# zkHubHQ/distributed-groth16

Hardware: NVIDIA H100
Metric: G1 MSM throughput (BN254 Pippenger, 2^20 pairs per GPU) (higher is better)
Workload: dtype u32x8 Montgomery (256-bit modular integers)

## Files before the change

### distributed_groth16_b200/csrc/ec.cuh

```cuda
#pragma once
#include "fp.cuh"

namespace b200zk {

template <class F>
struct affine_t {
    F x, y;
    B2_HD bool is_inf() const { return x.is_zero() && y.is_zero(); }
    B2_HD static affine_t infinity() { affine_t r; r.x = F::zero(); r.y = F::zero(); return r; }
};

template <class F>
struct xyzz_t {
    F x, y, zz, zzz;

    B2_HD static xyzz_t identity() {
        xyzz_t r; r.x = F::zero(); r.y = F::zero(); r.zz = F::zero(); r.zzz = F::zero(); return r;
    }
    B2_HD bool is_inf() const { return zz.is_zero(); }

    B2_HD static xyzz_t from_affine(const affine_t<F>& p) {
        if (p.is_inf()) return identity();
        xyzz_t r; r.x = p.x; r.y = p.y; r.zz = F::one(); r.zzz = F::one(); return r;
    }
// ... 138 lines not shown
        return r;
    }
    B2_HD_NI static affine_t<F> to_affine(const xyzz_t& a) {
        if (a.is_inf()) return affine_t<F>::infinity();
        return to_affine(a, F::inv(a.zzz));
    }

    B2_HD_NI static xyzz_t mul_scalar(const xyzz_t& p, const uint32_t k[8]) {
        xyzz_t acc = identity();
        for (int bit = 255; bit >= 0; --bit) {
            acc = dbl(acc);
            if ((k[bit >> 5] >> (bit & 31)) & 1) acc = add(acc, p);
        }
        return acc;
    }
};

template <class F> B2_HD affine_t<F> curve_generator();
template <> B2_HD affine_t<Fq> curve_generator<Fq>() {
    affine_t<Fq> g;
    for (int i = 0; i < 8; ++i) { g.x.l[i] = CurveConst::g1_gen_x(i); g.y.l[i] = CurveConst::g1_gen_y(i); }
    return g;
}
template <> B2_HD affine_t<Fq2> curve_generator<Fq2>() {
    affine_t<Fq2> g;
    for (int i = 0; i < 8; ++i) {
        g.x.c0.l[i] = CurveConst::g2_gen_x0(i); g.x.c1.l[i] = CurveConst::g2_gen_x1(i);
        g.y.c0.l[i] = CurveConst::g2_gen_y0(i); g.y.c1.l[i] = CurveConst::g2_gen_y1(i);
    }
    return g;
}

#ifdef __CUDACC__
template <class F, bool FULLWARP = false>
struct quad_ops {
    static constexpr int WORDS = sizeof(F) / 4;

    __device__ __forceinline__ static unsigned quad_mask() { return FULLWARP ? 0xFFFFFFFFu : (0xFu << (threadIdx.x & 28u)); }
    __device__ __forceinline__ static int quad_lane() { return threadIdx.x & 3; }

    struct xch_t { F p[2][4]; };
    __device__ __forceinline__ static F sel(int q, const F& a0, const F& a1, const F& a2, const F& a3) {
        F r;
        const uint32_t* p0 = reinterpret_cast<const uint32_t*>(&a0);
        const uint32_t* p1 = reinterpret_cast<const uint32_t*>(&a1);
        const uint32_t* p2 = reinterpret_cast<const uint32_t*>(&a2);
        const uint32_t* p3 = reinterpret_cast<const uint32_t*>(&a3);
        uint32_t* pr = reinterpret_cast<uint32_t*>(&r);
#pragma unroll
        for (int i = 0; i < WORDS; ++i) pr[i] = q == 0 ? p0[i] : q == 1 ? p1[i] : q == 2 ? p2[i] : p3[i];
        return r;
    }
    __device__ __forceinline__ static void mul4(xch_t* x, int buf, const F& a0, const F& b0, const F& a1, const F& b1,
                                                const F& a2, const F& b2, const F& a3, const F& b3, F& p0, F& p1, F& p2, F& p3) {
        const int q = quad_lane();
        F a = sel(q, a0, a1, a2, a3), b = sel(q, b0, b1, b2, b3);
        F p = F::mul(a, b);
        st16(&x->p[buf][q], p);
        __syncwarp(quad_mask());
        p0 = ld16(&x->p[buf][0]); p1 = ld16(&x->p[buf][1]); p2 = ld16(&x->p[buf][2]); p3 = ld16(&x->p[buf][3]);
    }

    __device__ static xyzz_t<F> dbl(xch_t* x, const xyzz_t<F>& p) {
        if (p.is_inf()) return p;
        F U = F::dbl(p.y);
        F V, X2, d0, d1;
        mul4(x, 0, U, U, p.x, p.x, U, U, U, U, V, X2, d0, d1);
        F M = F::add(F::dbl(X2), X2);
        F W, S, ZZ3, MM;
        mul4(x, 1, U, V, p.x, V, V, p.zz, M, M, W, S, ZZ3, MM);
        xyzz_t<F> r;
        r.x = F::sub(MM, F::dbl(S));
        F T1, T2, ZZZ3;
        mul4(x, 0, M, F::sub(S, r.x), W, p.y, W, p.zzz, W, W, T1, T2, ZZZ3, d0);
        r.y = F::sub(T1, T2);
        r.zz = ZZ3;
        r.zzz = ZZZ3;
        __syncwarp(quad_mask());
        return r;
    }

    __device__ static xyzz_t<F> add(xch_t* x, const xyzz_t<F>& a, const xyzz_t<F>& b) {
        if (a.is_inf()) return b;
        if (b.is_inf()) return a;
        F U1, U2, S1, S2;
        mul4(x, 0, a.x, b.zz, b.x, a.zz, a.y, b.zzz, b.y, a.zzz, U1, U2, S1, S2);
        F Pp = F::sub(U2, U1), R = F::sub(S2, S1);
        if (Pp.is_zero()) {
            __syncwarp(quad_mask());
            if (R.is_zero()) return dbl(x, a);
            return xyzz_t<F>::identity();
        }
        F PP, RR, ZZ12, ZZZ12;
        mul4(x, 1, Pp, Pp, R, R, a.zz, b.zz, a.zzz, b.zzz, PP, RR, ZZ12, ZZZ12);
        F PPP, Q, ZZ3, d0;
        mul4(x, 0, Pp, PP, U1, PP, ZZ12, PP, PP, PP, PPP, Q, ZZ3, d0);
        xyzz_t<F> r;
        r.x = F::sub(F::sub(RR, PPP), F::dbl(Q));
        F T1, T2, ZZZ3;
        mul4(x, 1, R, F::sub(Q, r.x), S1, PPP, ZZZ12, PPP, PPP, PPP, T1, T2, ZZZ3, d0);
        r.y = F::sub(T1, T2);
        r.zz = ZZ3;
        r.zzz = ZZZ3;
        __syncwarp(quad_mask());
        return r;
    }
};
#endif

struct G1Curve {
    typedef Fq F;
    static constexpr int LIMBS64 = 8;
};
struct G2Curve {
    typedef Fq2 F;
    static constexpr int LIMBS64 = 16;
};

}
```

### distributed_groth16_b200/csrc/msm.cu

```cuda
#include "common.cuh"
#include "glv.cuh"

namespace b200zk {

static const uint32_t KEY_NONE = 0xFFFFFFFFu;

__global__ void k_msm_digits(const Fr* scalars, uint32_t n, uint32_t c, uint32_t W, uint32_t* keys, uint32_t* ranks,
                             uint32_t* counts) {
    uint32_t i = blockIdx.x * blockDim.x + threadIdx.x;
    if (i >= n) return;
    Fr s = Fr::from_mont(ld16(scalars + i));
    uint32_t k[9];
#pragma unroll
    for (int j = 0; j < 8; ++j) k[j] = s.l[j];
    k[8] = 0;
    const uint32_t B = 1u << (c - 1);
    const uint32_t mask = (1u << c) - 1;
    uint32_t carry = 0;
    for (uint32_t w = 0; w < W; ++w) {
        uint32_t off = w * c, limb = off >> 5, sh = off & 31;
        uint64_t v = limb < 8 ? ((uint64_t)k[limb] | ((uint64_t)k[limb + 1] << 32)) : 0;
        uint32_t d = ((uint32_t)(v >> sh) & mask) + carry;
        uint32_t key = KEY_NONE, rank = 0;
        carry = 0;
        uint32_t neg = 0;
        if (d > B) { d = (1u << c) - d; neg = 1; carry = 1; }
        if (d != 0) {
            uint32_t g = d - 1;
            rank = atomicAdd(counts + g, 1u);
            key = g | (neg << 31);
        }
        const size_t slot = (size_t)w * n + i;
        keys[slot] = key;
        ranks[slot] = rank;
// ... 288 lines not shown
        run = Q::add(x, run, ld16(bw + k));
        acc = Q::add(x, acc, run);
    }
    if (lo) {
        xyzz_t<F> m = xyzz_t<F>::identity();
        for (int bit = 31 - __clz(lo); bit >= 0; --bit) {
            m = Q::dbl(x, m);
            if ((lo >> bit) & 1) m = Q::add(x, m, run);
        }
        acc = Q::add(x, acc, m);
    }
    if ((threadIdx.x & 3) == 0) st16(partials + t, acc);
}

template <class F, int THREADS>
__global__ void __launch_bounds__(THREADS) k_msm_window_sum(const xyzz_t<F>* partials, uint32_t nseg, xyzz_t<F>* wsum) {
    __shared__ xyzz_t<F> sh[THREADS];
    const xyzz_t<F>* p = partials + (size_t)blockIdx.x * nseg;
    xyzz_t<F> acc = xyzz_t<F>::identity();
    for (uint32_t i = threadIdx.x; i < nseg; i += THREADS) acc = add_sel<F>(acc, ld16(p + i));
    sh[threadIdx.x] = acc;
    __syncthreads();
    for (int s = THREADS / 2; s > 0; s >>= 1) {
        if ((int)threadIdx.x < s) {
            xyzz_t<F> a = sh[threadIdx.x], b = sh[threadIdx.x + s];
            sh[threadIdx.x] = add_sel<F>(a, b);
        }
        __syncthreads();
    }
    if (threadIdx.x == 0) st16(wsum + blockIdx.x, sh[0]);
}

template <class F>
__global__ void __launch_bounds__(32) k_msm_horner(const xyzz_t<F>* wsum, uint32_t nset, uint32_t c, uint32_t first, uint32_t last,
                                                   xyzz_t<F>* state, xyzz_t<F>* out) {
    typedef quad_ops<F, false> Q;
    __shared__ typename Q::xch_t xch;
    if (blockIdx.x != 0 || threadIdx.x >= 4) return;
    xyzz_t<F> total;
    uint32_t k = 0;
    if (first) { total = ld16(wsum); k = 1; }
    else total = ld16(state);
    for (; k < nset; ++k) {
        for (uint32_t j = 0; j < c; ++j) total = Q::dbl(&xch, total);
        total = Q::add(&xch, total, ld16(wsum + k));
    }
    if (threadIdx.x == 0) st16(last ? out : state, total);
}

template <class F>
__global__ void __launch_bounds__(32) k_msm_horner_glv(const xyzz_t<F>* wsum, uint32_t nwin, uint32_t c, uint32_t first, uint32_t last,
                                                       xyzz_t<F>* state, xyzz_t<F>* out) {
    typedef quad_ops<F, false> Q;
    __shared__ typename Q::xch_t xch[2];
    __shared__ xyzz_t<F> h1;
    if (blockIdx.x != 0 || threadIdx.x >= 8) return;
    const uint32_t half = threadIdx.x >> 2;
    xyzz_t<F> total;
    uint32_t k = 0;
    if (first) { total = ld16(wsum + half); k = 1; }
    else total = ld16(state + half);
    for (; k < nwin; ++k) {
        for (uint32_t j = 0; j < c; ++j) total = Q::dbl(&xch[half], total);
        total = Q::add(&xch[half], total, ld16(wsum + 2 * k + half));
    }
    if (!last) {
        if ((threadIdx.x & 3) == 0) st16(state + half, total);
        return;
    }
    if (threadIdx.x == 4) h1 = total;
    __syncwarp(0xFFu);
    if (half == 0) {
        xyzz_t<F> p = h1;
        if (!p.is_inf()) glv_phi_x(p.x);
        total = Q::add(&xch[0], total, p);
        if (threadIdx.x == 0) st16(out, total);
    }
}

template <class F>
__global__ void k_sum_to_affine(const xyzz_t<F>* pts, uint32_t count, affine_t<F>* out, uint64_t* flag) {
    if (threadIdx.x != 0 || blockIdx.x != 0) return;
    xyzz_t<F> acc = xyzz_t<F>::identity();
    for (uint32_t i = 0; i < count; ++i) acc = xyzz_t<F>::add(acc, ld16(pts + i));
    affine_t<F> a = xyzz_t<F>::to_affine(acc);
    st16(out, a);
    *flag = acc.is_inf() ? 1 : 0;
}

template <class F>
__global__ void k_set_identity(xyzz_t<F>* out) {
    if (threadIdx.x == 0 && blockIdx.x == 0) st16(out, xyzz_t<F>::identity());
}

static unsigned choose_window(size_t n) {
    unsigned lg = ceil_log2(n < 2 ? 2 : n);
    int c = (int)lg - 4;
    if (c < 5) c = 5;
    if (c > 20) c = 20;
    const char* env = getenv("B200ZK_MSM_WINDOW");
    if (env) { int v = atoi(env); if (v >= 2 && v <= 24) c = v; }
    return (unsigned)c;
}

// ... 39 lines not shown
template <class F>
static int msm_dev_impl(b200zk_ctx* ctx, const MsmStreams& ms, DevBuf& ws_buf, const MsmPart* parts, unsigned nparts,
                        void* d_out, const char* acc_name, unsigned tab_c = 0) {
    const int ch = ms.channel;
    size_t nev = 0;
    auto next_event = [&]() { return msm_event(ctx, ch, nev++); };
    size_t n = 0, n_max = 0;
    for (unsigned p = 0; p < nparts; ++p) { n += parts[p].n; n_max = parts[p].n > n_max ? parts[p].n : n_max; }
    xyzz_t<F>* out = reinterpret_cast<xyzz_t<F>*>(d_out);
    if (n == 0) {
        {
            LaunchScope ls(ctx, ms.acc, "msm_small");
            k_set_identity<F><<<1, 32, 0, ms.acc>>>(out);
        }
        return check_launch(ctx, "k_set_identity");
    }
    if (n >= (1ull << 31)) return set_error(ctx, B200ZK_ERR_ARG, "MSM length must be < 2^31");
    const bool fold = tab_c != 0;
    if (fold && nparts != 1) return set_error(ctx, B200ZK_ERR_ARG, "fixed-base tables take one input part");
    const unsigned c = fold ? tab_c : choose_window(n);
    const unsigned Wh = (128 + c - 1) / c;
    const unsigned W = fold ? msm_table_windows(c) : 2 * Wh;
    const unsigned WB = fold ? 1 : W;
    if ((uint64_t)W * n >= (fold ? (1ull << 31) : (1ull << 32)))
        return set_error(ctx, B200ZK_ERR_ARG, "MSM too large for 32-bit bucket offsets / entry indices (W * n)");
    const uint32_t B = 1u << (c - 1);
    const uint32_t nb = WB * B;
    uint32_t seg_len = B < 16 ? B : 16;
    const bool quad_reduce = (uint64_t)WB * (B / seg_len) <= 8192;
    if (quad_reduce) seg_len = B < 8 ? B : 8;
    else if (ctx->msm_seg_hint && ctx->msm_seg_hint <= B) seg_len = ctx->msm_seg_hint;
    const uint32_t nseg = B / seg_len;
    const uint32_t wsplit = fold ? (nseg >= 16 * 256 ? 16 : (nseg >= 1024 ? 4 : 1)) : 1;

    const unsigned unit_sets = fold ? 1 : 2;
    const unsigned units = fold ? 1 : Wh;
    unsigned ngroups = 1;
    if (!fold && nparts == 1 && n >= (1u << 22)) ngroups = units < 4 ? units : 4;
    auto group_first_unit = [&](unsigned g) { return (unsigned)(((uint64_t)units * g) / ngroups); };
    const uint32_t rmw = nparts > 1 ? 1u : 0u;

    const bool split_streams = ngroups > 1 || nparts > 1;
    const cudaStream_t st = split_streams ? ms.seq : ms.acc, ast = ms.acc;
    if (split_streams) {
        cudaEvent_t e = next_event();
        if (!e) return set_error(ctx, B200ZK_ERR_CUDA, "cudaEventCreate failed");
        B2_CUDA_OK(ctx, cudaEventRecord(e, ast));
        B2_CUDA_OK(ctx, cudaStreamWaitEvent(st, e, 0));
    }
    auto finish = [&]() -> int {
        if (split_streams) {
            cudaEvent_t e = next_event();
            if (!e) return set_error(ctx, B200ZK_ERR_CUDA, "cudaEventCreate failed");
            B2_CUDA_OK(ctx, cudaEventRecord(e, st));
            B2_CUDA_OK(ctx, cudaStreamWaitEvent(ast, e, 0));
        }
        return B200ZK_OK;
    };

    auto al = [](size_t x) { return (x + 255) & ~(size_t)255; };
    const size_t total_max = (size_t)W * n_max;
    uint32_t task_len = TASK_LEN;
    while (task_len < MAX_TASK_LEN && (uint64_t)task_len * nb < 3 * (uint64_t)total_max &&
           total_max / (2 * task_len) + nb >= (1u << 19))
        task_len *= 2;
    if (n_max <= (1u << 16))
        while (task_len > 16 && total_max / task_len < (1u << 17)) task_len /= 2;
    const size_t max_tasks = total_max / task_len + nb + ngroups;
    size_t o = 0;
    auto carve = [&](size_t bytes) { size_t r = o; o += al(bytes); return r; };
    struct PartWs { size_t keys, ranks, entries, counts, offsets, ntasks, taskoff, taskbucket, multi, hist, rank, order, tasksums; };
    std::vector<PartWs> pw(nparts);
    for (unsigned p = 0; p < nparts; ++p) {
        const size_t total = (size_t)W * parts[p].n;
        pw[p].keys = carve(total * 4); pw[p].ranks = carve(total * 4); pw[p].entries = carve(total * 4);
        pw[p].counts = carve(((size_t)nb + 1) * 4); pw[p].offsets = carve(((size_t)nb + 1) * 4);
        pw[p].ntasks = carve(((size_t)nb + ngroups) * 4); pw[p].taskoff = carve(((size_t)nb + ngroups) * 4);
        pw[p].taskbucket = carve(max_tasks * 4);
        pw[p].multi = carve((total_max / task_len + 4 * ngroups + 4) * 4);
        pw[p].hist = carve((size_t)ngroups * (MAX_TASK_LEN + 1) * 4);
        pw[p].rank = carve(max_tasks * 4); pw[p].order = carve(max_tasks * 4);
        pw[p].tasksums = carve(max_tasks * sizeof(xyzz_t<F>));
    }
    const size_t o_sums = carve(((size_t)nb / SCAN_TILE + 2) * 4);
    const size_t o_buckets = carve((size_t)nb * sizeof(xyzz_t<F>));
    const size_t o_partials = carve((size_t)WB * nseg * sizeof(xyzz_t<F>));
    const size_t o_wsum = carve((size_t)WB * wsplit * sizeof(xyzz_t<F>));
    const size_t o_state = carve(2 * sizeof(xyzz_t<F>));
    B2_CUDA_OK(ctx, ws_buf.reserve(o));
    char* ws = reinterpret_cast<char*>(ws_buf.p);
    uint32_t* sums = reinterpret_cast<uint32_t*>(ws + o_sums);
    xyzz_t<F>* buckets = reinterpret_cast<xyzz_t<F>*>(ws + o_buckets);
    xyzz_t<F>* partials = reinterpret_cast<xyzz_t<F>*>(ws + o_partials);
    xyzz_t<F>* wsum = reinterpret_cast<xyzz_t<F>*>(ws + o_wsum);
    xyzz_t<F>* hstate = reinterpret_cast<xyzz_t<F>*>(ws + o_state);
    B2_CUDA_OK(ctx, cudaMemsetAsync(buckets, 0, (size_t)nb * sizeof(xyzz_t<F>), st));
    cudaEvent_t buckets_clear = nullptr;
    if (rmw) {
        buckets_clear = next_event();
        if (!buckets_clear) return set_error(ctx, B200ZK_ERR_CUDA, "cudaEventCreate failed");
        B2_CUDA_OK(ctx, cudaEventRecord(buckets_clear, st));
        B2_CUDA_OK(ctx, cudaStreamWaitEvent(ast, buckets_clear, 0));
    }

    struct Group {
        uint32_t set0, nsets, b0, nbk;
        size_t task_cap, task_base;
        uint32_t list_cap; size_t list_base;
    };
    std::vector<Group> groups(ngroups);
    {
        size_t tb = 0, lb = 2 * (size_t)ngroups;
        for (unsigned g = 0; g < ngroups; ++g) {
            Group& G = groups[g];
            const unsigned u0 = group_first_unit(g), u1 = group_first_unit(g + 1);
            G.set0 = u0 * unit_sets; G.nsets = (u1 - u0) * unit_sets;
            G.b0 = G.set0 * B; G.nbk = G.nsets * B;
            const size_t gtotal = fold ? total_max : (size_t)G.nsets * n_max;
            G.task_cap = gtotal / task_len + G.nbk + 1;
            G.task_base = tb; tb += G.task_cap;
// ... 116 lines not shown
        }
    }
    for (unsigned g = 0; g < ngroups; ++g) {
        const Group& G = groups[g];
        for (unsigned p = 0; p < nparts; ++p) B2_CUDA_OK(ctx, cudaStreamWaitEvent(st, accumulated[(size_t)p * ngroups + g], 0));
        if (!rmw) {
            uint32_t* multi_all = reinterpret_cast<uint32_t*>(ws + pw[0].multi);
            uint32_t* task_off = reinterpret_cast<uint32_t*>(ws + pw[0].taskoff) + G.b0 + g;
            xyzz_t<F>* task_sums = reinterpret_cast<xyzz_t<F>*>(ws + pw[0].tasksums) + G.task_base;
            {
                LaunchScope ls(ctx, st, "msm_merge");
                k_msm_merge_tasks<F><<<2 * ctx->sm_count, 128, 0, st>>>(multi_all + G.list_base, multi_all + 2 * g, task_off, task_sums, 0u, buckets + G.b0);
            }
            {
                LaunchScope ls(ctx, st, "msm_merge");
                k_msm_merge_small<F><<<4 * ctx->sm_count, 128, 0, st>>>(multi_all + G.list_base, G.list_cap, multi_all + 2 * g + 1, task_off, task_sums,
                                                                       0u, buckets + G.b0);
            }
            B2_TRY(check_launch(ctx, "k_msm_merge_tasks"));
        }
        {
            LaunchScope ls(ctx, st, "msm_reduce");
            if (quad_reduce)
                k_msm_reduce_segments_quad<F><<<(G.nsets * nseg * 4 + 127) / 128, 128, 0, st>>>(buckets + G.b0, G.nsets, B, seg_len,
                                                                                               partials + (size_t)G.set0 * nseg);
            else
                k_msm_reduce_segments<F><<<(G.nsets * nseg + 127) / 128, 128, 0, st>>>(buckets + G.b0, G.nsets, B, seg_len,
                                                                                      partials + (size_t)G.set0 * nseg);
        }
        B2_TRY(check_launch(ctx, "k_msm_reduce_segments"));
        {
            LaunchScope ls(ctx, st, "msm_window_sum");
            constexpr int T = sizeof(F) > 32 ? 128 : 256;
            k_msm_window_sum<F, T><<<G.nsets * wsplit, T, 0, st>>>(partials + (size_t)G.set0 * nseg, nseg / wsplit, wsum + (size_t)G.set0 * wsplit);
        }
        B2_TRY(check_launch(ctx, "k_msm_window_sum"));
        {
            LaunchScope ls(ctx, st, "msm_combine");
            const uint32_t first = g == 0, last = g + 1 == ngroups;
            if (fold) k_msm_horner<F><<<1, 32, 0, st>>>(wsum, wsplit, 0u, first, last, hstate, out);
            else k_msm_horner_glv<F><<<1, 32, 0, st>>>(wsum + G.set0, G.nsets / 2, c, first, last, hstate, out);
        }
        B2_TRY(check_launch(ctx, "k_msm_horner"));
    }
    return finish();
}

template <class F>
static int msm_dev_impl(b200zk_ctx* ctx, const MsmStreams& ms, DevBuf& ws_buf, const void* d_bases, const void* d_scalars, size_t n,
                        void* d_out, const char* acc_name, cudaEvent_t bases_ready, cudaEvent_t scalars_ready = nullptr,
                        unsigned tab_c = 0) {
    const MsmPart part{d_bases, d_scalars, n, bases_ready, scalars_ready};
    return msm_dev_impl<F>(ctx, ms, ws_buf, &part, 1, d_out, acc_name, tab_c);
}

static MsmStreams slot_streams(b200zk_ctx* ctx, Slot& sl, int aux) {
    const int ch = 2 * (int)(&sl - ctx->slots) + (aux ? 1 : 0);
    return MsmStreams{ctx->msm_side[ch], aux ? sl.aux_stream : sl.stream, ch};
}

int msm_g1_dev(b200zk_ctx* ctx, Slot& sl, const void* d_bases, const void* d_scalars, size_t n, void* d_out,
               cudaEvent_t bases_ready, int aux) {
    return msm_dev_impl<Fq>(ctx, slot_streams(ctx, sl, aux), aux ? sl.ws_msm_aux : sl.ws_msm, d_bases, d_scalars, n, d_out,
                            "msm_accumulate_g1", bases_ready);
}
int msm_g2_dev(b200zk_ctx* ctx, Slot& sl, const void* d_bases, const void* d_scalars, size_t n, void* d_out,
               cudaEvent_t bases_ready, int aux) {
    return msm_dev_impl<Fq2>(ctx, slot_streams(ctx, sl, aux), aux ? sl.ws_msm_aux : sl.ws_msm, d_bases, d_scalars, n, d_out,
                             "msm_accumulate_g2", bases_ready);
}

unsigned msm_table_windows(unsigned c) { return (255 + c - 1) / c; }
unsigned msm_table_auto_window(size_t n) {
    int L = (int)ceil_log2(n < 2 ? 2 : n);
// ... 236 lines not shown
```

### distributed_groth16_b200/csrc/selftest.cu

```cuda
#include <type_traits>

#include "codec.cuh"
#include "glv.cuh"
#include "pairing.cuh"
#ifdef __CUDACC__
#include "common.cuh"
#endif

namespace b200zk {

enum {
    ARITH_FQ = 0, ARITH_FR = 32,
    FP_ADD = 0, FP_SUB, FP_NEG, FP_DBL, FP_MUL, FP_MUL_NI, FP_SQR, FP_MUL_ANY, FP_MUL_K2, FP_MUL_K3, FP_MUL_K4,
    FP_MUL_WIDE_REDC1, FP_REDC2, FP_INV, FP_INV_FERMAT, FP_TO_MONT, FP_FROM_MONT, FP_FROM_U32, FP_POW_U64,
    ARITH_FR_ROOT = 64,
    ARITH_FQ2_MUL = 70, ARITH_FQ2_SQR, ARITH_FQ2_INV, ARITH_FQ2_MUL_GROUP1, ARITH_FQ2_MUL_GROUP2, ARITH_FQ2_MUL_GROUP3,
    ARITH_FQ2_MUL_GROUP4, ARITH_FQ2_MUL_XI, ARITH_FQ2_CONJ, ARITH_GLV_PHI_G1, ARITH_GLV_PHI_G2,
    ARITH_FQ_POW_P1_4 = 84, ARITH_FQ_SQRT, ARITH_FQ2_SQRT, ARITH_FQ_HALF, ARITH_FQ_IS_LARGER, ARITH_FQ2_IS_LARGER,
    ARITH_FQ_FROM_BYTES,
    ARITH_FQ6_MUL = 96, ARITH_FQ6_INV, ARITH_FQ6_MUL_V, ARITH_FQ12_MUL, ARITH_FQ12_INV, ARITH_FQ12_CONJ, ARITH_FQ12_FROB2,
    ARITH_FINAL_EXP, ARITH_PAIRING, ARITH_G2_FROBENIUS_TWIST,
    ARITH_GLV_DECOMPOSE = 108,
    ARITH_G1 = 112, ARITH_G2 = 128,
    EC_DBL = 0, EC_ADD, EC_DBL_ILP, EC_ADD_ILP, EC_MADD, EC_DBL_AFFINE, EC_TO_AFFINE, EC_MUL_SCALAR,
    EC_QUAD_ADD, EC_QUAD_DBL, EC_QUAD_ADD_FULLWARP, EC_QUAD_DBL_FULLWARP,
};

#define B2_ARITH_FP_OPS(X, B)                                                                                             \
    X(B + FP_ADD, 8, 4) X(B + FP_SUB, 8, 4) X(B + FP_NEG, 4, 4) X(B + FP_DBL, 4, 4) X(B + FP_MUL, 8, 4)                   \
    X(B + FP_MUL_NI, 8, 4) X(B + FP_SQR, 4, 4) X(B + FP_MUL_ANY, 8, 4) X(B + FP_MUL_K2, 16, 8) X(B + FP_MUL_K3, 24, 12)   \
    X(B + FP_MUL_K4, 32, 16) X(B + FP_MUL_WIDE_REDC1, 8, 12) X(B + FP_REDC2, 8, 4) X(B + FP_INV, 4, 4)                   \
    X(B + FP_INV_FERMAT, 4, 4) X(B + FP_TO_MONT, 4, 4) X(B + FP_FROM_MONT, 4, 4) X(B + FP_FROM_U32, 1, 4)                \
    X(B + FP_POW_U64, 5, 4)
#define B2_ARITH_EC_OPS(X, B, W)                                                                                          \
    X(B + EC_DBL, 4 * W, 4 * W) X(B + EC_ADD, 8 * W, 4 * W) X(B + EC_DBL_ILP, 4 * W, 4 * W) X(B + EC_ADD_ILP, 8 * W, 4 * W) \
    X(B + EC_MADD, 6 * W + 1, 4 * W) X(B + EC_DBL_AFFINE, 2 * W, 4 * W) X(B + EC_TO_AFFINE, 4 * W, 2 * W)                \
    X(B + EC_MUL_SCALAR, 4 * W + 4, 4 * W)
#define B2_ARITH_OPS(X)                                                                                                   \
    B2_ARITH_FP_OPS(X, ARITH_FQ) B2_ARITH_FP_OPS(X, ARITH_FR)                                                             \
    X(ARITH_FQ2_MUL, 16, 8) X(ARITH_FQ2_SQR, 8, 8) X(ARITH_FQ2_INV, 8, 8) X(ARITH_FQ2_MUL_GROUP1, 16, 8)                  \
    X(ARITH_FQ2_MUL_GROUP2, 32, 16) X(ARITH_FQ2_MUL_GROUP3, 48, 24) X(ARITH_FQ2_MUL_GROUP4, 64, 32)                      \
    X(ARITH_FQ2_MUL_XI, 8, 8) X(ARITH_FQ2_CONJ, 8, 8) X(ARITH_GLV_PHI_G1, 4, 4) X(ARITH_GLV_PHI_G2, 8, 8)                 \
    X(ARITH_FQ_POW_P1_4, 4, 4) X(ARITH_FQ_SQRT, 4, 5) X(ARITH_FQ2_SQRT, 8, 9) X(ARITH_FQ_HALF, 4, 4)                      \
    X(ARITH_FQ_IS_LARGER, 4, 1) X(ARITH_FQ2_IS_LARGER, 8, 1) X(ARITH_FQ_FROM_BYTES, 5, 5)                                \
    X(ARITH_FQ6_MUL, 48, 24) X(ARITH_FQ6_INV, 24, 24) X(ARITH_FQ6_MUL_V, 24, 24) X(ARITH_FQ12_MUL, 96, 48)                \
    X(ARITH_FQ12_INV, 48, 48) X(ARITH_FQ12_CONJ, 48, 48) X(ARITH_FQ12_FROB2, 48, 48) X(ARITH_FINAL_EXP, 48, 48)           \
    X(ARITH_PAIRING, 24, 48) X(ARITH_G2_FROBENIUS_TWIST, 16, 16) X(ARITH_GLV_DECOMPOSE, 4, 6)                            \
    B2_ARITH_EC_OPS(X, ARITH_G1, 4) B2_ARITH_EC_OPS(X, ARITH_G2, 8)
#define B2_ARITH_DEVICE_OPS(X)                                                                                            \
    X(ARITH_FR_ROOT, 1, 4)                                                                                                \
    X(ARITH_G1 + EC_QUAD_ADD, 32, 16) X(ARITH_G1 + EC_QUAD_DBL, 16, 16) X(ARITH_G1 + EC_QUAD_ADD_FULLWARP, 32, 16)       \
    X(ARITH_G1 + EC_QUAD_DBL_FULLWARP, 16, 16) X(ARITH_G2 + EC_QUAD_ADD, 64, 32) X(ARITH_G2 + EC_QUAD_DBL, 32, 32)       \
    X(ARITH_G2 + EC_QUAD_ADD_FULLWARP, 64, 32) X(ARITH_G2 + EC_QUAD_DBL_FULLWARP, 32, 32)

B2_HD void arith_words(int op, int* in, int* out) {
    *in = 0; *out = 0;
    switch (op) {
#define B2_ARITH_WORDS(OP, IN, OUT) case OP: *in = IN; *out = OUT; break;
        B2_ARITH_OPS(B2_ARITH_WORDS)
        B2_ARITH_DEVICE_OPS(B2_ARITH_WORDS)
#undef B2_ARITH_WORDS
        default: break;
    }
}

template <class T>
B2_HD T arith_ld(const uint64_t* w) {
    T r;
    uint32_t* d = reinterpret_cast<uint32_t*>(&r);
    for (int i = 0; i < (int)(sizeof(T) / 4); ++i) d[i] = (uint32_t)(w[i >> 1] >> (32 * (i & 1)));
    return r;
}
template <class T>
B2_HD void arith_st(uint64_t* w, const T& v) {
    const uint32_t* s = reinterpret_cast<const uint32_t*>(&v);
    for (int i = 0; i < (int)(sizeof(T) / 8); ++i) w[i] = (uint64_t)s[2 * i] | (uint64_t)s[2 * i + 1] << 32;
}
B2_HD void arith_st_limbs(uint64_t* w, const uint32_t* l, int n32) {
    for (int i = 0; i < n32 / 2; ++i) w[i] = (uint64_t)l[2 * i] | (uint64_t)l[2 * i + 1] << 32;
}

template <class F, int S>
B2_HD void arith_fp(const uint64_t* in, uint64_t* out) {
    if constexpr (S == FP_ADD) arith_st(out, F::add(arith_ld<F>(in), arith_ld<F>(in + 4)));
    else if constexpr (S == FP_SUB) arith_st(out, F::sub(arith_ld<F>(in), arith_ld<F>(in + 4)));
    else if constexpr (S == FP_NEG) arith_st(out, F::neg(arith_ld<F>(in)));
// ... 120 lines not shown
}

#ifdef __CUDACC__
constexpr int ARITH_BLOCK = 128;

template <int OP>
__global__ void __launch_bounds__(ARITH_BLOCK) k_arith(const uint64_t* in, uint64_t* out, size_t n, int in_w, int out_w) {
    const size_t i = (size_t)blockIdx.x * blockDim.x + threadIdx.x;
    if (i >= n) return;
    arith_apply<OP>(in + i * in_w, out + i * out_w);
}

__global__ void __launch_bounds__(ARITH_BLOCK) k_arith_fr_root(const uint64_t* in, uint64_t* out, size_t n) {
    const size_t i = (size_t)blockIdx.x * blockDim.x + threadIdx.x;
    if (i >= n) return;
    arith_st(out + 4 * i, fr_root_of_unity((unsigned)(in[i] & 0xFF), ((in[i] >> 8) & 1) != 0));
}

template <class F, bool FULLWARP, bool DBL>
__global__ void __launch_bounds__(ARITH_BLOCK) k_arith_quad(const uint64_t* in, uint64_t* out, size_t n) {
    typedef quad_ops<F, FULLWARP> Q;
    typedef xyzz_t<F> X;
    constexpr int XW = (int)sizeof(X) / 8;
    __shared__ __align__(16) typename Q::xch_t xch[ARITH_BLOCK / 4];
    const size_t t = (size_t)blockIdx.x * blockDim.x + threadIdx.x;
    const size_t i = FULLWARP ? t >> 5 : t >> 2;
    if (i >= n) return;
    typename Q::xch_t* x = &xch[threadIdx.x >> 2];
    const uint64_t* r = in + i * (DBL ? XW : 2 * XW);
    const X res = DBL ? Q::dbl(x, arith_ld<X>(r)) : Q::add(x, arith_ld<X>(r), arith_ld<X>(r + XW));
    if ((threadIdx.x & (FULLWARP ? 31u : 3u)) == 0) arith_st(out + i * XW, res);
}

static int arith_launch(b200zk_ctx* ctx, Slot& sl, int op, const uint64_t* d_in, uint64_t* d_out, size_t n, int in_w,
                        int out_w) {
    const unsigned grid1 = (unsigned)((n + ARITH_BLOCK - 1) / ARITH_BLOCK);
    const unsigned grid4 = (unsigned)((4 * n + ARITH_BLOCK - 1) / ARITH_BLOCK);
    const unsigned grid32 = (unsigned)((32 * n + ARITH_BLOCK - 1) / ARITH_BLOCK);
    LaunchScope ls(ctx, sl.stream, "arith");
    switch (op) {
#define B2_ARITH_CASE(OP, IN, OUT) \
        case OP: k_arith<OP><<<grid1, ARITH_BLOCK, 0, sl.stream>>>(d_in, d_out, n, in_w, out_w); break;
        B2_ARITH_OPS(B2_ARITH_CASE)
#undef B2_ARITH_CASE
        case ARITH_FR_ROOT: k_arith_fr_root<<<grid1, ARITH_BLOCK, 0, sl.stream>>>(d_in, d_out, n); break;
        case ARITH_G1 + EC_QUAD_ADD: k_arith_quad<Fq, false, false><<<grid4, ARITH_BLOCK, 0, sl.stream>>>(d_in, d_out, n); break;
        case ARITH_G1 + EC_QUAD_DBL: k_arith_quad<Fq, false, true><<<grid4, ARITH_BLOCK, 0, sl.stream>>>(d_in, d_out, n); break;
        case ARITH_G1 + EC_QUAD_ADD_FULLWARP: k_arith_quad<Fq, true, false><<<grid32, ARITH_BLOCK, 0, sl.stream>>>(d_in, d_out, n); break;
        case ARITH_G1 + EC_QUAD_DBL_FULLWARP: k_arith_quad<Fq, true, true><<<grid32, ARITH_BLOCK, 0, sl.stream>>>(d_in, d_out, n); break;
        case ARITH_G2 + EC_QUAD_ADD: k_arith_quad<Fq2, false, false><<<grid4, ARITH_BLOCK, 0, sl.stream>>>(d_in, d_out, n); break;
        case ARITH_G2 + EC_QUAD_DBL: k_arith_quad<Fq2, false, true><<<grid4, ARITH_BLOCK, 0, sl.stream>>>(d_in, d_out, n); break;
        case ARITH_G2 + EC_QUAD_ADD_FULLWARP: k_arith_quad<Fq2, true, false><<<grid32, ARITH_BLOCK, 0, sl.stream>>>(d_in, d_out, n); break;
        case ARITH_G2 + EC_QUAD_DBL_FULLWARP: k_arith_quad<Fq2, true, true><<<grid32, ARITH_BLOCK, 0, sl.stream>>>(d_in, d_out, n); break;
        default: return set_error(ctx, B200ZK_ERR_ARG, "b200zk_test_arith: no such op");
    }
    return check_launch(ctx, "k_arith");
}
#endif

}

#ifdef __CUDACC__
using namespace b200zk;

extern "C" int b200zk_test_arith(b200zk_ctx* ctx, int op, const uint64_t* in, size_t n, uint64_t* out) {
    int in_w, out_w;
    arith_words(op, &in_w, &out_w);
    if (!ctx || in_w == 0) return set_error(ctx, B200ZK_ERR_ARG, "b200zk_test_arith: no such op");
    if (n == 0) return B200ZK_OK;
    if (!in || !out) return B200ZK_ERR_ARG;
    Slot& sl = ctx->slots[0];
    std::lock_guard<std::mutex> g(sl.mu);
    B2_CUDA_OK(ctx, cudaSetDevice(ctx->device));
    const size_t in_bytes = n * in_w * 8, out_bytes = n * out_w * 8;
    B2_CUDA_OK(ctx, sl.io_a.reserve(in_bytes + out_bytes + 64));
    uint64_t* d_in = reinterpret_cast<uint64_t*>(sl.io_a.p);
    uint64_t* d_out = d_in + n * in_w;
    B2_CUDA_OK(ctx, cudaMemcpyAsync(d_in, in, in_bytes, cudaMemcpyHostToDevice, sl.stream));
    B2_CUDA_OK(ctx, cudaMemsetAsync(d_out, 0xFF, out_bytes, sl.stream));
    B2_TRY(arith_launch(ctx, sl, op, d_in, d_out, n, in_w, out_w));
    B2_CUDA_OK(ctx, cudaMemcpyAsync(out, d_out, out_bytes, cudaMemcpyDeviceToHost, sl.stream));
    B2_CUDA_OK(ctx, cudaStreamSynchronize(sl.stream));
    return B200ZK_OK;
}
#endif
```

Before: 221.7.

## Add 8-lane-per-multiply G1 group law for Horner and split window sums

```diff
diff --git a/distributed_groth16_b200/csrc/ec.cuh b/distributed_groth16_b200/csrc/ec.cuh
--- a/distributed_groth16_b200/csrc/ec.cuh
+++ b/distributed_groth16_b200/csrc/ec.cuh
@@ -194,12 +194,63 @@
 }
 
 #ifdef __CUDACC__
+template <class F, class M>
+struct coop_group_law {
+    template <class X>
+    __device__ static xyzz_t<F> dbl(X* x, const xyzz_t<F>& p) {
+        if (p.is_inf()) return p;
+        F U = F::dbl(p.y);
+        F V, X2, d0, d1;
+        M::mul4(x, 0, U, U, p.x, p.x, U, U, U, U, V, X2, d0, d1);
+        F Mm = F::add(F::dbl(X2), X2);
+        F W, S, ZZ3, MM;
+        M::mul4(x, 1, U, V, p.x, V, V, p.zz, Mm, Mm, W, S, ZZ3, MM);
+        xyzz_t<F> r;
+        r.x = F::sub(MM, F::dbl(S));
+        F T1, T2, ZZZ3;
+        M::mul4(x, 0, Mm, F::sub(S, r.x), W, p.y, W, p.zzz, W, W, T1, T2, ZZZ3, d0);
+        r.y = F::sub(T1, T2);
+        r.zz = ZZ3;
+        r.zzz = ZZZ3;
+        M::sync();
+        return r;
+    }
+
+    template <class X>
+    __device__ static xyzz_t<F> add(X* x, const xyzz_t<F>& a, const xyzz_t<F>& b) {
+        if (a.is_inf()) return b;
+        if (b.is_inf()) return a;
+        F U1, U2, S1, S2;
+        M::mul4(x, 0, a.x, b.zz, b.x, a.zz, a.y, b.zzz, b.y, a.zzz, U1, U2, S1, S2);
+        F Pp = F::sub(U2, U1), R = F::sub(S2, S1);
+        if (Pp.is_zero()) {
+            M::sync();
+            if (R.is_zero()) return dbl(x, a);
+            return xyzz_t<F>::identity();
+        }
+        F PP, RR, ZZ12, ZZZ12;
+        M::mul4(x, 1, Pp, Pp, R, R, a.zz, b.zz, a.zzz, b.zzz, PP, RR, ZZ12, ZZZ12);
+        F PPP, Q, ZZ3, d0;
+        M::mul4(x, 0, Pp, PP, U1, PP, ZZ12, PP, PP, PP, PPP, Q, ZZ3, d0);
+        xyzz_t<F> r;
+        r.x = F::sub(F::sub(RR, PPP), F::dbl(Q));
+        F T1, T2, ZZZ3;
+        M::mul4(x, 1, R, F::sub(Q, r.x), S1, PPP, ZZZ12, PPP, PPP, PPP, T1, T2, ZZZ3, d0);
+        r.y = F::sub(T1, T2);
+        r.zz = ZZ3;
+        r.zzz = ZZZ3;
+        M::sync();
+        return r;
+    }
+};
+
 template <class F, bool FULLWARP = false>
-struct quad_ops {
+struct quad_ops : coop_group_law<F, quad_ops<F, FULLWARP>> {
     static constexpr int WORDS = sizeof(F) / 4;
 
     __device__ __forceinline__ static unsigned quad_mask() { return FULLWARP ? 0xFFFFFFFFu : (0xFu << (threadIdx.x & 28u)); }
     __device__ __forceinline__ static int quad_lane() { return threadIdx.x & 3; }
+    __device__ __forceinline__ static void sync() { __syncwarp(quad_mask()); }
 
     struct xch_t { F p[2][4]; };
     __device__ __forceinline__ static F sel(int q, const F& a0, const F& a1, const F& a2, const F& a3) {
@@ -222,51 +273,6 @@
         __syncwarp(quad_mask());
         p0 = ld16(&x->p[buf][0]); p1 = ld16(&x->p[buf][1]); p2 = ld16(&x->p[buf][2]); p3 = ld16(&x->p[buf][3]);
     }
-
-    __device__ static xyzz_t<F> dbl(xch_t* x, const xyzz_t<F>& p) {
-        if (p.is_inf()) return p;
-        F U = F::dbl(p.y);
-        F V, X2, d0, d1;
-        mul4(x, 0, U, U, p.x, p.x, U, U, U, U, V, X2, d0, d1);
-        F M = F::add(F::dbl(X2), X2);
-        F W, S, ZZ3, MM;
-        mul4(x, 1, U, V, p.x, V, V, p.zz, M, M, W, S, ZZ3, MM);
-        xyzz_t<F> r;
-        r.x = F::sub(MM, F::dbl(S));
-        F T1, T2, ZZZ3;
-        mul4(x, 0, M, F::sub(S, r.x), W, p.y, W, p.zzz, W, W, T1, T2, ZZZ3, d0);
-        r.y = F::sub(T1, T2);
-        r.zz = ZZ3;
-        r.zzz = ZZZ3;
-        __syncwarp(quad_mask());
-        return r;
-    }
-
-    __device__ static xyzz_t<F> add(xch_t* x, const xyzz_t<F>& a, const xyzz_t<F>& b) {
-        if (a.is_inf()) return b;
-        if (b.is_inf()) return a;
-        F U1, U2, S1, S2;
-        mul4(x, 0, a.x, b.zz, b.x, a.zz, a.y, b.zzz, b.y, a.zzz, U1, U2, S1, S2);
-        F Pp = F::sub(U2, U1), R = F::sub(S2, S1);
-        if (Pp.is_zero()) {
-            __syncwarp(quad_mask());
-            if (R.is_zero()) return dbl(x, a);
-            return xyzz_t<F>::identity();
-        }
-        F PP, RR, ZZ12, ZZZ12;
-        mul4(x, 1, Pp, Pp, R, R, a.zz, b.zz, a.zzz, b.zzz, PP, RR, ZZ12, ZZZ12);
-        F PPP, Q, ZZ3, d0;
-        mul4(x, 0, Pp, PP, U1, PP, ZZ12, PP, PP, PP, PPP, Q, ZZ3, d0);
-        xyzz_t<F> r;
-        r.x = F::sub(F::sub(RR, PPP), F::dbl(Q));
-        F T1, T2, ZZZ3;
-        mul4(x, 1, R, F::sub(Q, r.x), S1, PPP, ZZZ12, PPP, PPP, PPP, T1, T2, ZZZ3, d0);
-        r.y = F::sub(T1, T2);
-        r.zz = ZZ3;
-        r.zzz = ZZZ3;
-        __syncwarp(quad_mask());
-        return r;
-    }
 };
 #endif
 
diff --git a/distributed_groth16_b200/csrc/lane8.cuh b/distributed_groth16_b200/csrc/lane8.cuh
--- /dev/null
+++ b/distributed_groth16_b200/csrc/lane8.cuh
@@ -0,0 +1,80 @@
+#pragma once
+#include "ec.cuh"
+
+namespace b200zk {
+#ifdef __CUDACC__
+
+template <class F>
+struct lane8_ops;
+
+template <class P>
+struct lane8_ops<Fp<P>> : coop_group_law<Fp<P>, lane8_ops<Fp<P>>> {
+    typedef Fp<P> F;
+    static constexpr unsigned FULL = 0xFFFFFFFFu;
+
+    __device__ __forceinline__ static uint32_t pick(const uint32_t (&v)[8], int j) {
+        uint32_t r = v[0];
+#pragma unroll
+        for (int k = 1; k < 8; ++k) r = j == k ? v[k] : r;
+        return r;
+    }
+    __device__ __forceinline__ static uint32_t mod_limb(int j) {
+        uint32_t r = P::mod(0);
+#pragma unroll
+        for (int k = 1; k < 8; ++k) r = j == k ? P::mod(k) : r;
+        return r;
+    }
+
+    __device__ __forceinline__ static uint32_t mul_limb(const F& a, const F& b) {
+        const int j = threadIdx.x & 7;
+        const unsigned octet = threadIdx.x & 24u;
+        const uint32_t aj = pick(a.l, j), pj = mod_limb(j);
+        uint32_t l = 0, h = 0, t = 0;
+        uint32_t zl = 0, zh = 0, zt = 0;
+#pragma unroll
+        for (int i = 0; i < 8; ++i) {
+            l = cc::mad_lo_cc(aj, b.l[i], l); h = cc::madc_hi_cc(aj, b.l[i], h); t = cc::addc(t, 0);
+            zl = cc::mad_lo_cc(a.l[0], b.l[i], zl); zh = cc::madc_hi_cc(a.l[0], b.l[i], zh); zt = cc::addc(zt, 0);
+            const uint32_t m = zl * P::INV;
+            l = cc::mad_lo_cc(m, pj, l); h = cc::madc_hi_cc(m, pj, h); t = cc::addc(t, 0);
+            zl = cc::mad_lo_cc(m, P::mod(0), zl); zh = cc::madc_hi_cc(m, P::mod(0), zh); zt = cc::addc(zt, 0);
+            uint32_t down = __shfl_down_sync(FULL, l, 1, 8);
+            const uint32_t l1 = __shfl_sync(FULL, l, 1, 8);
+            down = j == 7 ? 0u : down;
+            l = cc::add_cc(h, down); h = cc::addc(t, 0); t = 0;
+            zl = cc::add_cc(zh, l1); zh = cc::addc(zt, 0); zt = 0;
+        }
+        uint32_t hu = __shfl_up_sync(FULL, h, 1, 8);
+        hu = j == 0 ? 0u : hu;
+        const uint32_t w = cc::add_cc(l, hu);
+        const uint32_t g = cc::addc(0, 0);
+        const uint32_t G = (__ballot_sync(FULL, g != 0) >> octet) & 0xFFu;
+        const uint32_t Pr = (__ballot_sync(FULL, w == 0xFFFFFFFFu) >> octet) & 0xFFu;
+        const uint32_t r = w + (((Pr + (G << 1)) ^ Pr) >> j & 1u);
+        const uint32_t d = cc::sub_cc(r, pj);
+        const uint32_t bg = cc::subc(0, 0) & 1u;
+        const uint32_t BG = (__ballot_sync(FULL, bg != 0) >> octet) & 0xFFu;
+        const uint32_t BP = (__ballot_sync(FULL, r == pj) >> octet) & 0xFFu;
+        const uint32_t bin = (BP + (BG << 1)) ^ BP;
+        return (bin >> 8) & 1u ? r : d - (bin >> j & 1u);
+    }
+
+    struct xch_t { F p[2][4]; };
+    __device__ __forceinline__ static F sel(unsigned k, const F& a0, const F& a1, const F& a2, const F& a3) {
+        F r;
+#pragma unroll
+        for (int i = 0; i < 8; ++i) r.l[i] = k == 0 ? a0.l[i] : k == 1 ? a1.l[i] : k == 2 ? a2.l[i] : a3.l[i];
+        return r;
+    }
+    __device__ __forceinline__ static void sync() { __syncwarp(); }
+    __device__ __forceinline__ static void mul4(xch_t* x, int buf, const F& a0, const F& b0, const F& a1, const F& b1,
+                                                const F& a2, const F& b2, const F& a3, const F& b3, F& p0, F& p1, F& p2, F& p3) {
+        const unsigned k = (threadIdx.x >> 3) & 3u;
+        x->p[buf][k].l[threadIdx.x & 7] = mul_limb(sel(k, a0, a1, a2, a3), sel(k, b0, b1, b2, b3));
+        __syncwarp();
+        p0 = ld16(&x->p[buf][0]); p1 = ld16(&x->p[buf][1]); p2 = ld16(&x->p[buf][2]); p3 = ld16(&x->p[buf][3]);
+    }
+};
+
+#endif
+}
diff --git a/distributed_groth16_b200/csrc/msm.cu b/distributed_groth16_b200/csrc/msm.cu
--- a/distributed_groth16_b200/csrc/msm.cu
+++ b/distributed_groth16_b200/csrc/msm.cu
@@ -1,5 +1,8 @@
 #include "common.cuh"
 #include "glv.cuh"
+#include "lane8.cuh"
+
+#include <type_traits>
 
 namespace b200zk {
 
@@ -354,6 +357,24 @@
 }
 
 template <class F>
+__global__ void __launch_bounds__(32) k_msm_window_join(const xyzz_t<F>* part, uint32_t parts, xyzz_t<F>* wsum) {
+    typedef quad_ops<F, false> Q;
+    __shared__ __align__(16) typename Q::xch_t xch[8];
+    __shared__ __align__(16) xyzz_t<F> sh[8];
+    const uint32_t q = threadIdx.x >> 2;
+    const xyzz_t<F>* p = part + (size_t)blockIdx.x * parts;
+    xyzz_t<F> acc = xyzz_t<F>::identity();
+    for (uint32_t i = q; i < parts; i += 8) acc = Q::add(&xch[q], acc, ld16(p + i));
+    for (uint32_t s = 4; s > 0; s >>= 1) {
+        if ((threadIdx.x & 3) == 0) st16(&sh[q], acc);
+        __syncwarp();
+        if (q < s) acc = Q::add(&xch[q], acc, ld16(&sh[q + s]));
+        __syncwarp();
+    }
+    if (threadIdx.x == 0) st16(wsum + blockIdx.x, acc);
+}
+
+template <class F>
 __global__ void __launch_bounds__(32) k_msm_horner(const xyzz_t<F>* wsum, uint32_t nset, uint32_t c, uint32_t first, uint32_t last,
                                                    xyzz_t<F>* state, xyzz_t<F>* out) {
     typedef quad_ops<F, false> Q;
@@ -371,13 +392,15 @@
 }
 
 template <class F>
-__global__ void __launch_bounds__(32) k_msm_horner_glv(const xyzz_t<F>* wsum, uint32_t nwin, uint32_t c, uint32_t first, uint32_t last,
+__global__ void __launch_bounds__(64) k_msm_horner_glv(const xyzz_t<F>* wsum, uint32_t nwin, uint32_t c, uint32_t first, uint32_t last,
                                                        xyzz_t<F>* state, xyzz_t<F>* out) {
-    typedef quad_ops<F, false> Q;
-    __shared__ typename Q::xch_t xch[2];
+    constexpr bool LANE8 = sizeof(F) == 32;
+    typedef typename std::conditional<LANE8, lane8_ops<Fq>, quad_ops<F, false>>::type Q;
+    constexpr unsigned SHIFT = LANE8 ? 5 : 2;
+    __shared__ __align__(16) typename Q::xch_t xch[2];
     __shared__ xyzz_t<F> h1;
-    if (blockIdx.x != 0 || threadIdx.x >= 8) return;
-    const uint32_t half = threadIdx.x >> 2;
+    if (blockIdx.x != 0 || threadIdx.x >= (2u << SHIFT)) return;
+    const uint32_t half = threadIdx.x >> SHIFT, lead = threadIdx.x & ((1u << SHIFT) - 1);
     xyzz_t<F> total;
     uint32_t k = 0;
     if (first) { total = ld16(wsum + half); k = 1; }
@@ -387,11 +410,11 @@
         total = Q::add(&xch[half], total, ld16(wsum + 2 * k + half));
     }
     if (!last) {
-        if ((threadIdx.x & 3) == 0) st16(state + half, total);
+        if (lead == 0) st16(state + half, total);
         return;
     }
-    if (threadIdx.x == 4) h1 = total;
-    __syncwarp(0xFFu);
+    if (threadIdx.x == (1u << SHIFT)) h1 = total;
+    if (LANE8) __syncthreads(); else __syncwarp(0xFFu);
     if (half == 0) {
         xyzz_t<F> p = h1;
         if (!p.is_inf()) glv_phi_x(p.x);
@@ -497,6 +520,7 @@
     else if (ctx->msm_seg_hint && ctx->msm_seg_hint <= B) seg_len = ctx->msm_seg_hint;
     const uint32_t nseg = B / seg_len;
     const uint32_t wsplit = fold ? (nseg >= 16 * 256 ? 16 : (nseg >= 1024 ? 4 : 1)) : 1;
+    const uint32_t wpart = (!fold && sizeof(F) == 32 && nseg >= 1024) ? 16 : 1;
 
     const unsigned unit_sets = fold ? 1 : 2;
     const unsigned units = fold ? 1 : Wh;
@@ -550,7 +574,7 @@
     const size_t o_sums = carve(((size_t)nb / SCAN_TILE + 2) * 4);
     const size_t o_buckets = carve((size_t)nb * sizeof(xyzz_t<F>));
     const size_t o_partials = carve((size_t)WB * nseg * sizeof(xyzz_t<F>));
-    const size_t o_wsum = carve((size_t)WB * wsplit * sizeof(xyzz_t<F>));
+    const size_t o_wsum = carve((size_t)WB * (wsplit + (wpart > 1 ? wpart : 0)) * sizeof(xyzz_t<F>));
     const size_t o_state = carve(2 * sizeof(xyzz_t<F>));
     B2_CUDA_OK(ctx, ws_buf.reserve(o));
     char* ws = reinterpret_cast<char*>(ws_buf.p);
@@ -733,14 +757,20 @@
         {
             LaunchScope ls(ctx, st, "msm_window_sum");
             constexpr int T = sizeof(F) > 32 ? 128 : 256;
-            k_msm_window_sum<F, T><<<G.nsets * wsplit, T, 0, st>>>(partials + (size_t)G.set0 * nseg, nseg / wsplit, wsum + (size_t)G.set0 * wsplit);
+            if (wpart > 1) {
+                xyzz_t<F>* wpartial = wsum + (size_t)WB * wsplit + (size_t)G.set0 * wpart;
+                k_msm_window_sum<F, 128><<<G.nsets * wpart, 128, 0, st>>>(partials + (size_t)G.set0 * nseg, nseg / wpart, wpartial);
+                k_msm_window_join<F><<<G.nsets, 32, 0, st>>>(wpartial, wpart, wsum + G.set0);
+            } else {
+                k_msm_window_sum<F, T><<<G.nsets * wsplit, T, 0, st>>>(partials + (size_t)G.set0 * nseg, nseg / wsplit, wsum + (size_t)G.set0 * wsplit);
+            }
         }
         B2_TRY(check_launch(ctx, "k_msm_window_sum"));
         {
             LaunchScope ls(ctx, st, "msm_combine");
             const uint32_t first = g == 0, last = g + 1 == ngroups;
             if (fold) k_msm_horner<F><<<1, 32, 0, st>>>(wsum, wsplit, 0u, first, last, hstate, out);
-            else k_msm_horner_glv<F><<<1, 32, 0, st>>>(wsum + G.set0, G.nsets / 2, c, first, last, hstate, out);
+            else k_msm_horner_glv<F><<<1, 64, 0, st>>>(wsum + G.set0, G.nsets / 2, c, first, last, hstate, out);
         }
         B2_TRY(check_launch(ctx, "k_msm_horner"));
     }
diff --git a/distributed_groth16_b200/csrc/selftest.cu b/distributed_groth16_b200/csrc/selftest.cu
--- a/distributed_groth16_b200/csrc/selftest.cu
+++ b/distributed_groth16_b200/csrc/selftest.cu
@@ -5,6 +5,7 @@
 #include "pairing.cuh"
 #ifdef __CUDACC__
 #include "common.cuh"
+#include "lane8.cuh"
 #endif
 
 namespace b200zk {
@@ -24,6 +25,7 @@
     ARITH_G1 = 112, ARITH_G2 = 128,
     EC_DBL = 0, EC_ADD, EC_DBL_ILP, EC_ADD_ILP, EC_MADD, EC_DBL_AFFINE, EC_TO_AFFINE, EC_MUL_SCALAR,
     EC_QUAD_ADD, EC_QUAD_DBL, EC_QUAD_ADD_FULLWARP, EC_QUAD_DBL_FULLWARP,
+    ARITH_LANE8_FQ_MUL = 144, ARITH_LANE8_G1_ADD, ARITH_LANE8_G1_DBL, ARITH_CHAIN_G1_LANE8, ARITH_CHAIN_G1_QUAD,
 };
 
 #define B2_ARITH_FP_OPS(X, B)                                                                                             \
@@ -52,6 +54,9 @@
     X(ARITH_G1 + EC_QUAD_ADD, 32, 16) X(ARITH_G1 + EC_QUAD_DBL, 16, 16) X(ARITH_G1 + EC_QUAD_ADD_FULLWARP, 32, 16)       \
     X(ARITH_G1 + EC_QUAD_DBL_FULLWARP, 16, 16) X(ARITH_G2 + EC_QUAD_ADD, 64, 32) X(ARITH_G2 + EC_QUAD_DBL, 32, 32)       \
     X(ARITH_G2 + EC_QUAD_ADD_FULLWARP, 64, 32) X(ARITH_G2 + EC_QUAD_DBL_FULLWARP, 32, 32)
+#define B2_ARITH_LANE8_OPS(X)                                                                                             \
+    X(ARITH_LANE8_FQ_MUL, 8, 4) X(ARITH_LANE8_G1_ADD, 32, 16) X(ARITH_LANE8_G1_DBL, 16, 16)                              \
+    X(ARITH_CHAIN_G1_LANE8, 32, 16) X(ARITH_CHAIN_G1_QUAD, 32, 16)
 
 B2_HD void arith_words(int op, int* in, int* out) {
     *in = 0; *out = 0;
@@ -238,10 +243,54 @@
     if ((threadIdx.x & (FULLWARP ? 31u : 3u)) == 0) arith_st(out + i * XW, res);
 }
 
+__global__ void __launch_bounds__(ARITH_BLOCK) k_arith_lane8_mul(const uint64_t* in, uint64_t* out, size_t n) {
+    typedef lane8_ops<Fq> L;
+    const size_t t = (size_t)blockIdx.x * blockDim.x + threadIdx.x;
+    const size_t i = t >> 3 < n ? t >> 3 : n - 1;
+    const uint32_t limb = L::mul_limb(arith_ld<Fq>(in + 8 * i), arith_ld<Fq>(in + 8 * i + 4));
+    if (t >> 3 < n) reinterpret_cast<uint32_t*>(out + 4 * i)[t & 7] = limb;
+}
+
+constexpr int CHAIN_WINDOWS = 8, CHAIN_C = 16;
+template <class Q>
+__device__ __forceinline__ xyzz_t<Fq> arith_chain(typename Q::xch_t* x, xyzz_t<Fq> acc, const xyzz_t<Fq>& q) {
+    for (int w = 1; w < CHAIN_WINDOWS; ++w) {
+        for (int j = 0; j < CHAIN_C; ++j) acc = Q::dbl(x, acc);
+        acc = Q::add(x, acc, q);
+    }
+    return Q::add(x, acc, q);
+}
+
+template <int OP>
+__global__ void __launch_bounds__(ARITH_BLOCK) k_arith_lane8_ec(const uint64_t* in, uint64_t* out, size_t n) {
+    typedef lane8_ops<Fq> L;
+    typedef xyzz_t<Fq> X;
+    __shared__ __align__(16) typename L::xch_t xch[ARITH_BLOCK / 32];
+    const size_t w = ((size_t)blockIdx.x * blockDim.x + threadIdx.x) >> 5;
+    if (w >= n) return;
+    typename L::xch_t* x = &xch[threadIdx.x >> 5];
+    const uint64_t* r = in + w * (OP == ARITH_LANE8_G1_DBL ? 16 : 32);
+    X res;
+    if constexpr (OP == ARITH_LANE8_G1_DBL) res = L::dbl(x, arith_ld<X>(r));
+    else if constexpr (OP == ARITH_LANE8_G1_ADD) res = L::add(x, arith_ld<X>(r), arith_ld<X>(r + 16));
+    else res = arith_chain<L>(x, arith_ld<X>(r), arith_ld<X>(r + 16));
+    if ((threadIdx.x & 31) == 0) arith_st(out + w * 16, res);
+}
+
+__global__ void __launch_bounds__(ARITH_BLOCK) k_arith_chain_quad(const uint64_t* in, uint64_t* out, size_t n) {
+    typedef quad_ops<Fq, false> Q;
+    __shared__ __align__(16) typename Q::xch_t xch[ARITH_BLOCK / 4];
+    const size_t i = ((size_t)blockIdx.x * blockDim.x + threadIdx.x) >> 2;
+    if (i >= n) return;
+    const xyzz_t<Fq> res = arith_chain<Q>(&xch[threadIdx.x >> 2], arith_ld<xyzz_t<Fq>>(in + 32 * i), arith_ld<xyzz_t<Fq>>(in + 32 * i + 16));
+    if ((threadIdx.x & 3) == 0) arith_st(out + 16 * i, res);
+}
+
 static int arith_launch(b200zk_ctx* ctx, Slot& sl, int op, const uint64_t* d_in, uint64_t* d_out, size_t n, int in_w,
                         int out_w) {
     const unsigned grid1 = (unsigned)((n + ARITH_BLOCK - 1) / ARITH_BLOCK);
     const unsigned grid4 = (unsigned)((4 * n + ARITH_BLOCK - 1) / ARITH_BLOCK);
+    const unsigned grid8 = (unsigned)((8 * n + ARITH_BLOCK - 1) / ARITH_BLOCK);
     const unsigned grid32 = (unsigned)((32 * n + ARITH_BLOCK - 1) / ARITH_BLOCK);
     LaunchScope ls(ctx, sl.stream, "arith");
     switch (op) {
@@ -258,6 +307,11 @@
         case ARITH_G2 + EC_QUAD_DBL: k_arith_quad<Fq2, false, true><<<grid4, ARITH_BLOCK, 0, sl.stream>>>(d_in, d_out, n); break;
         case ARITH_G2 + EC_QUAD_ADD_FULLWARP: k_arith_quad<Fq2, true, false><<<grid32, ARITH_BLOCK, 0, sl.stream>>>(d_in, d_out, n); break;
         case ARITH_G2 + EC_QUAD_DBL_FULLWARP: k_arith_quad<Fq2, true, true><<<grid32, ARITH_BLOCK, 0, sl.stream>>>(d_in, d_out, n); break;
+        case ARITH_LANE8_FQ_MUL: k_arith_lane8_mul<<<grid8, ARITH_BLOCK, 0, sl.stream>>>(d_in, d_out, n); break;
+        case ARITH_LANE8_G1_ADD: k_arith_lane8_ec<ARITH_LANE8_G1_ADD><<<grid32, ARITH_BLOCK, 0, sl.stream>>>(d_in, d_out, n); break;
+        case ARITH_LANE8_G1_DBL: k_arith_lane8_ec<ARITH_LANE8_G1_DBL><<<grid32, ARITH_BLOCK, 0, sl.stream>>>(d_in, d_out, n); break;
+        case ARITH_CHAIN_G1_LANE8: k_arith_lane8_ec<ARITH_CHAIN_G1_LANE8><<<grid32, ARITH_BLOCK, 0, sl.stream>>>(d_in, d_out, n); break;
+        case ARITH_CHAIN_G1_QUAD: k_arith_chain_quad<<<grid4, ARITH_BLOCK, 0, sl.stream>>>(d_in, d_out, n); break;
         default: return set_error(ctx, B200ZK_ERR_ARG, "b200zk_test_arith: no such op");
     }
     return check_launch(ctx, "k_arith");
@@ -272,6 +326,12 @@
 extern "C" int b200zk_test_arith(b200zk_ctx* ctx, int op, const uint64_t* in, size_t n, uint64_t* out) {
     int in_w, out_w;
     arith_words(op, &in_w, &out_w);
+    switch (op) {
+#define B2_ARITH_WORDS(OP, IN, OUT) case OP: in_w = IN; out_w = OUT; break;
+        B2_ARITH_LANE8_OPS(B2_ARITH_WORDS)
+#undef B2_ARITH_WORDS
+        default: break;
+    }
     if (!ctx || in_w == 0) return set_error(ctx, B200ZK_ERR_ARG, "b200zk_test_arith: no such op");
     if (n == 0) return B200ZK_OK;
     if (!in || !out) return B200ZK_ERR_ARG;
```

Measured after the change: 227.1, median of 6. +2.5%, better.
